# haoyuzhao123/CGRayTracing

Measured on NVIDIA B200. Metric: photons_per_s, higher is better.
Workload: dtype f64 decisions / f32 accumulators

## Files before the change

### cgraytracing_b200/csrc/cgrt_build.cuh

```cuda
#pragma once
#include "cgrt_device.cuh"

namespace cgrt {

#define RS_THREADS 256
#define RS_ITEMS 16
#define RS_TILE (RS_THREADS * RS_ITEMS)

template <typename K>
__global__ void __launch_bounds__(RS_THREADS) rs_hist_kernel(const K *__restrict__ keys, int64_t n, int shift, uint32_t *__restrict__ counts, int ntiles) {
    __shared__ uint32_t h[256];
    h[threadIdx.x] = 0;
    __syncthreads();
    int64_t base = (int64_t)blockIdx.x * RS_TILE;
#pragma unroll 4
    for (int r = 0; r < RS_ITEMS; r++) {
        int64_t i = base + r * RS_THREADS + threadIdx.x;
        if (i < n) atomicAdd(&h[(uint32_t)(keys[i] >> shift) & 255u], 1u);
    }
    __syncthreads();
    counts[(size_t)threadIdx.x * ntiles + blockIdx.x] = h[threadIdx.x];
}

__global__ void __launch_bounds__(1024) rs_scan_kernel(uint32_t *__restrict__ counts, int64_t m) {
    __shared__ uint32_t warp_sums[32];
    __shared__ uint32_t carry;
    if (threadIdx.x == 0) carry = 0;
    __syncthreads();
    int lane = threadIdx.x & 31, wid = threadIdx.x >> 5;
    for (int64_t base = 0; base < m; base += 1024) {
        int64_t i = base + threadIdx.x;
        uint32_t v = (i < m) ? counts[i] : 0u;
        uint32_t x = v;
#pragma unroll
        for (int o = 1; o < 32; o <<= 1) {
            uint32_t y = __shfl_up_sync(0xffffffffu, x, o);
            if (lane >= o) x += y;
        }
        if (lane == 31) warp_sums[wid] = x;
        __syncthreads();
        if (wid == 0) {
            uint32_t s = warp_sums[lane];
#pragma unroll
            for (int o = 1; o < 32; o <<= 1) {
                uint32_t y = __shfl_up_sync(0xffffffffu, s, o);
                if (lane >= o) s += y;
            }
            warp_sums[lane] = s;
        }
        __syncthreads();
        uint32_t prefix = carry + (wid > 0 ? warp_sums[wid - 1] : 0u) + x - v;
        if (i < m) counts[i] = prefix;
        __syncthreads();
        if (threadIdx.x == 1023) carry = prefix + v;
        __syncthreads();
    }
}

template <typename K>
__global__ void __launch_bounds__(RS_THREADS) rs_scatter_kernel(const K *__restrict__ keys_in, const uint32_t *__restrict__ vals_in,
                                                                K *__restrict__ keys_out, uint32_t *__restrict__ vals_out, int64_t n, int shift,
                                                                const uint32_t *__restrict__ offsets, int ntiles, int first_pass) {
    __shared__ uint32_t running[256];
    __shared__ uint32_t warp_cnt[RS_THREADS / 32][256];
    const int lane = threadIdx.x & 31, wid = threadIdx.x >> 5;
    running[threadIdx.x] = offsets[(size_t)threadIdx.x * ntiles + blockIdx.x];
#pragma unroll
    for (int w = 0; w < RS_THREADS / 32; w++) warp_cnt[w][threadIdx.x] = 0;
    __syncthreads();
    int64_t base = (int64_t)blockIdx.x * RS_TILE;
    for (int r = 0; r < RS_ITEMS; r++) {
        int64_t i = base + r * RS_THREADS + threadIdx.x;
        bool valid = i < n;
        K k = valid ? keys_in[i] : (K)0;
        uint32_t v = valid ? (first_pass ? (uint32_t)i : vals_in[i]) : 0u;
        uint32_t dg = valid ? ((uint32_t)(k >> shift) & 255u) : 256u;
        uint32_t mask = __match_any_sync(0xffffffffu, dg);
        uint32_t rank = __popc(mask & ((1u << lane) - 1u));
        if (valid && rank == 0) warp_cnt[wid][dg] = __popc(mask);
        __syncthreads();
        if (valid) {
            uint32_t pos = running[dg] + rank;
            for (int w = 0; w < wid; w++) pos += warp_cnt[w][dg];
            keys_out[pos] = k;
            vals_out[pos] = v;
        }
        __syncthreads();
        {
            uint32_t s = 0;
#pragma unroll
            for (int w = 0; w < RS_THREADS / 32; w++) { s += warp_cnt[w][threadIdx.x]; warp_cnt[w][threadIdx.x] = 0; }
            running[threadIdx.x] += s;
        }
        __syncthreads();
    }
}

__device__ __forceinline__ uint32_t float_flip(float f) {
    uint32_t u = __float_as_uint(f);
    return (u & 0x80000000u) ? ~u : (u | 0x80000000u);
}
__device__ __forceinline__ float float_unflip(uint32_t u) {
    return __uint_as_float((u & 0x80000000u) ? (u & 0x7fffffffu) : ~u);
}

__global__ void lbvh_bounds_kernel(const double *__restrict__ tri9, int n, uint32_t *__restrict__ bounds) {
    int i = blockIdx.x * blockDim.x + threadIdx.x;
    float c[3] = {3.0e38f, 3.0e38f, 3.0e38f}, C[3] = {-3.0e38f, -3.0e38f, -3.0e38f};
    if (i < n) {
        const double *t = tri9 + (size_t)i * 9;
        for (int a = 0; a < 3; a++) {
            float m = (float)((t[a] + t[3 + a] + t[6 + a]) * (1.0 / 3.0));
            c[a] = m; C[a] = m;
        }
    }
    for (int a = 0; a < 3; a++) {
        float lo = c[a], hi = C[a];
        for (int o = 16; o > 0; o >>= 1) {
            lo = fminf(lo, __shfl_xor_sync(0xffffffffu, lo, o));
            hi = fmaxf(hi, __shfl_xor_sync(0xffffffffu, hi, o));
        }
        if ((threadIdx.x & 31) == 0) {
            atomicMin(&bounds[a], float_flip(lo));
            atomicMax(&bounds[3 + a], float_flip(hi));
        }
    }
}

__device__ __forceinline__ uint32_t expand10(uint32_t v) {
    v = (v * 0x00010001u) & 0xFF0000FFu;
    v = (v * 0x00000101u) & 0x0F00F00Fu;
    v = (v * 0x00000011u) & 0xC30C30C3u;
    v = (v * 0x00000005u) & 0x49249249u;
    return v;
}

__global__ void lbvh_morton_kernel(const double *__restrict__ tri9, int n, const uint32_t *__restrict__ bounds, uint64_t *__restrict__ keys) {
    int i = blockIdx.x * blockDim.x + threadIdx.x;
    if (i >= n) return;
    const double *t = tri9 + (size_t)i * 9;
    uint32_t q[3];
    for (int a = 0; a < 3; a++) {
        float lo = float_unflip(bounds[a]), hi = float_unflip(bounds[3 + a]);
        float m = (float)((t[a] + t[3 + a] + t[6 + a]) * (1.0 / 3.0));
        float ext = hi - lo;
        float u = ext > 0.f ? (m - lo) / ext : 0.f;
        u = fminf(fmaxf(u * 1024.f, 0.f), 1023.f);
        q[a] = (uint32_t)u;
    }
    keys[i] = (uint64_t)((expand10(q[0]) << 2) | (expand10(q[1]) << 1) | expand10(q[2]));
}

__global__ void lbvh_leaves_kernel(const double *__restrict__ tri9, const uint32_t *__restrict__ perm, int n, TriRec *__restrict__ tris,
                                   int *__restrict__ tri_id, float *__restrict__ box ) {
    int k = blockIdx.x * blockDim.x + threadIdx.x;
    if (k >= n) return;
    uint32_t src = perm[k];
    const double *t = tri9 + (size_t)src * 9;
    d3 pa = mk(t[0], t[1], t[2]), pb = mk(t[3], t[4], t[5]), pc = mk(t[6], t[7], t[8]);
    d3 e1 = pa - pb, e2 = pa - pc;
    d3 nn = normalize(cross(pa - pb, pa - pc));
    TriRec R;
    R.pa[0] = pa.x; R.pa[1] = pa.y; R.pa[2] = pa.z;
    R.e1[0] = e1.x; R.e1[1] = e1.y; R.e1[2] = e1.z;
    R.e2[0] = e2.x; R.e2[1] = e2.y; R.e2[2] = e2.z;
    R.n[0] = nn.x; R.n[1] = nn.y; R.n[2] = nn.z;
    tris[k] = R;
    tri_id[k] = (int)src;
    float *b = box + (size_t)(n - 1 + k) * 6;
    const double pad = CGRT_BOX_PAD;
    for (int a = 0; a < 3; a++) {
        double lo = fmin(fmin(t[a], t[3 + a]), t[6 + a]), hi = fmax(fmax(t[a], t[3 + a]), t[6 + a]);
        b[a] = __double2float_rd(lo - pad - 1e-7 * fabs(lo));
        b[3 + a] = __double2float_ru(hi + pad + 1e-7 * fabs(hi));
    }
}

__device__ __forceinline__ int lbvh_delta(const uint64_t *__restrict__ keys, int n, int i, int j) {
    if (j < 0 || j >= n) return -1;
    uint64_t a = keys[i], b = keys[j];
    if (a == b) return 64 + __clz((uint32_t)i ^ (uint32_t)j);
    return __clzll((long long)(a ^ b));
}

__global__ void lbvh_hierarchy_kernel(const uint64_t *__restrict__ keys, int n, int *__restrict__ left, int *__restrict__ right, int *__restrict__ parent) {
    int i = blockIdx.x * blockDim.x + threadIdx.x;
    if (i >= n - 1) return;
    int d = (lbvh_delta(keys, n, i, i + 1) - lbvh_delta(keys, n, i, i - 1)) >= 0 ? 1 : -1;
    int dmin = lbvh_delta(keys, n, i, i - d);
    int lmax = 2;
    while (lbvh_delta(keys, n, i, i + lmax * d) > dmin) lmax <<= 1;
    int l = 0;
    for (int t = lmax >> 1; t >= 1; t >>= 1)
        if (lbvh_delta(keys, n, i, i + (l + t) * d) > dmin) l += t;
    int j = i + l * d;
    int dnode = lbvh_delta(keys, n, i, j);
    int s = 0;
    int t = l;
    do {
        t = (t + 1) >> 1;
        if (lbvh_delta(keys, n, i, i + (s + t) * d) > dnode) s += t;
    } while (t > 1);
    int gamma = i + s * d + min(d, 0);
    int lo = min(i, j), hi = max(i, j);
    int lc = (lo == gamma) ? (n - 1 + gamma) : gamma;
    int rc = (hi == gamma + 1) ? (n - 1 + gamma + 1) : (gamma + 1);
    left[i] = lc;
    right[i] = rc;
    parent[lc] = i;
    parent[rc] = i;
    if (i == 0) parent[0] = -1;
}

__global__ void lbvh_refit_kernel(int n, const int *__restrict__ left, const int *__restrict__ right, const int *__restrict__ parent,
                                  float *__restrict__ box, unsigned int *__restrict__ flags) {
    int k = blockIdx.x * blockDim.x + threadIdx.x;
    if (k >= n) return;
    int node = parent[n - 1 + k];
    while (node >= 0) {
        unsigned int old = atomicAdd(&flags[node], 1u);
        if (old == 0) return;
        __threadfence();
        const volatile float *a = box + (size_t)left[node] * 6;
        const volatile float *b = box + (size_t)right[node] * 6;
        float *o = box + (size_t)node * 6;
        for (int c = 0; c < 3; c++) {
            o[c] = fminf(a[c], b[c]);
            o[3 + c] = fmaxf(a[3 + c], b[3 + c]);
        }
        __threadfence();
        node = parent[node];
    }
}

__device__ __forceinline__ float lbvh_box_area(const float *__restrict__ b) {
    const float dx = b[3] - b[0], dy = b[4] - b[1], dz = b[5] - b[2];
    return dx * dy + dy * dz + dz * dx;
}
__global__ void lbvh_collapse_kernel(int n, int begin, int end, const int *__restrict__ left, const int *__restrict__ right, const float *__restrict__ box,
                                     int *__restrict__ queue, int *__restrict__ counter, BvhNode4 *__restrict__ nodes4) {
    int w = begin + blockIdx.x * blockDim.x + threadIdx.x;
    if (w >= end) return;
    const int b = queue[w];
    int c[4];
    int nc = 2;
    c[0] = left[b]; c[1] = right[b]; c[2] = -1; c[3] = -1;
    while (nc < 4) {
        int pick = -1;
        float best = -1.f;
        for (int j = 0; j < nc; j++) {
            if (c[j] >= n - 1) continue;
            float a = lbvh_box_area(box + (size_t)c[j] * 6);
            if (a > best) { best = a; pick = j; }
        }
        if (pick < 0) break;
        const int e = c[pick];
        c[pick] = left[e];
        c[nc++] = right[e];
    }
    for (int i = 1; i < nc; i++) {
        int v = c[i], j = i - 1;
        while (j >= 0 && c[j] > v) { c[j + 1] = c[j]; j--; }
        c[j + 1] = v;
    }
    BvhNode4 N;
    for (int j = 0; j < 4; j++) {
        if (j < nc) {
            const float *bb = box + (size_t)c[j] * 6;
            N.lox[j] = bb[0]; N.loy[j] = bb[1]; N.loz[j] = bb[2];
            N.hix[j] = bb[3]; N.hiy[j] = bb[4]; N.hiz[j] = bb[5];
            if (c[j] >= n - 1) {
                N.child[j] = ~(c[j] - (n - 1));
            } else {
                const int at = atomicAdd(counter, 1);
                queue[at] = c[j];
                N.child[j] = at;
            }
        } else {
            N.lox[j] = N.loy[j] = N.loz[j] = 3.0e38f;
            N.hix[j] = N.hiy[j] = N.hiz[j] = -3.0e38f;
            N.child[j] = CGRT_NO_CHILD;
        }
        N.pad[j] = 0;
    }
    nodes4[w] = N;
}

__global__ void bump_triangles_kernel(const double *__restrict__ height, int H, int W, double tex_px, double tex_pz, double lenx, double leny,
                                      double plane_y, double *__restrict__ tri9) {
    const int step = 3;
    int nj = W / step - 1, ni = H / step - 1;
    int idx = blockIdx.x * blockDim.x + threadIdx.x;
    if (idx >= ni * nj) return;
    int i = idx / nj, j = idx % nj;
    double x1 = tex_px + lenx * j * step / W;
    double x2 = tex_px + lenx * (j + 1) * step / W;
    double y1 = tex_pz + leny * i * step / H;
    double y2 = tex_pz + leny * (i + 1) * step / H;
    double ha = height[(size_t)(i * step) * W + j * step] + plane_y;
    double hb = height[(size_t)(i * step) * W + (j + 1) * step] + plane_y;
    double hc = height[(size_t)((i + 1) * step) * W + j * step] + plane_y;
    double hd = height[(size_t)((i + 1) * step) * W + (j + 1) * step] + plane_y;
    double *o = tri9 + (size_t)idx * 18;
    o[0] = x1; o[1] = ha; o[2] = y1;  o[3] = x2; o[4] = hb; o[5] = y1;  o[6] = x1; o[7] = hc; o[8] = y2;
    o[9] = x2; o[10] = hd; o[11] = y2;  o[12] = x2; o[13] = hb; o[14] = y1;  o[15] = x1; o[16] = hc; o[17] = y2;
}

__global__ void texture_stage_kernel(const uint8_t *__restrict__ rgb, int64_t ntexel, uchar4 *__restrict__ out) {
    int64_t i = (int64_t)blockIdx.x * blockDim.x + threadIdx.x;
    if (i >= ntexel) return;
    out[i] = make_uchar4(rgb[3 * i], rgb[3 * i + 1], rgb[3 * i + 2], 255);
}

}
```

### cgraytracing_b200/csrc/cgrt_device.cuh

```cuda
#pragma once
#include <cuda_runtime.h>
#include <stdint.h>

namespace cgrt {

struct d3 {
    double x, y, z;
};
__host__ __device__ __forceinline__ d3 mk(double x, double y, double z) { d3 r; r.x = x; r.y = y; r.z = z; return r; }
__host__ __device__ __forceinline__ d3 operator+(d3 a, d3 b) { return mk(a.x + b.x, a.y + b.y, a.z + b.z); }
__host__ __device__ __forceinline__ d3 operator-(d3 a, d3 b) { return mk(a.x - b.x, a.y - b.y, a.z - b.z); }
__host__ __device__ __forceinline__ d3 operator-(d3 a) { return mk(-a.x, -a.y, -a.z); }
__host__ __device__ __forceinline__ d3 operator*(d3 a, double f) { return mk(a.x * f, a.y * f, a.z * f); }
__host__ __device__ __forceinline__ d3 operator*(d3 a, d3 b) { return mk(a.x * b.x, a.y * b.y, a.z * b.z); }
__host__ __device__ __forceinline__ double dot(d3 a, d3 b) { return a.x * b.x + a.y * b.y + a.z * b.z; }
__host__ __device__ __forceinline__ d3 cross(d3 a, d3 b) {
    return mk(a.y * b.z - a.z * b.y, a.z * b.x - a.x * b.z, a.x * b.y - a.y * b.x);
}
__host__ __device__ __forceinline__ d3 normalize(d3 a) {
    double len = sqrt(a.x * a.x + a.y * a.y + a.z * a.z);
    if (len > 0) {
        a.x *= 1 / len;
        a.y *= 1 / len;
        a.z *= 1 / len;
    }
    return a;
}
__host__ __device__ __forceinline__ double det3(d3 a, d3 b, d3 c) {
    return (a.x * b.y * c.z + b.x * c.y * a.z + c.x * a.y * b.z - a.x * c.y * b.z - b.x * a.y * c.z - c.x * b.y * a.z);
}
__host__ __device__ __forceinline__ double max3(double a, double b, double c) {
    if (a > b && a > c) return a;
    else if (b > c) return b;
    else return c;
}

#define CGRT_EPS 1e-4
#define CGRT_INF 1e10
#define CGRT_PI 3.14159265358979

enum { PASS_EYE = 0, PASS_PHOTON = 1, PASS_BEZIER = 2, PASS_SPPM_EYE = 3 };

struct Philox {
    uint32_t k0, k1, c0, c1, c2, c3;
    uint32_t buf[4];
    int idx;
    __host__ __device__ __forceinline__ void init(uint64_t seed, uint32_t pass, uint64_t path, uint32_t dim) {
        k0 = (uint32_t)seed;
        k1 = (uint32_t)(seed >> 32) + pass;
        c0 = (uint32_t)path;
        c1 = (uint32_t)(path >> 32);
        c2 = dim;
        c3 = 0;
        idx = 4;
    }
    __host__ __device__ __forceinline__ void block() {
        uint32_t a0 = c0, a1 = c1, a2 = c2, a3 = c3, x0 = k0, x1 = k1;
#pragma unroll
        for (int r = 0; r < 10; r++) {
#ifdef __CUDA_ARCH__
            uint32_t h0 = __umulhi(0xD2511F53u, a0), l0 = 0xD2511F53u * a0;
            uint32_t h1 = __umulhi(0xCD9E8D57u, a2), l1 = 0xCD9E8D57u * a2;
#else
            uint64_t p0 = (uint64_t)0xD2511F53u * a0, p1 = (uint64_t)0xCD9E8D57u * a2;
            uint32_t h0 = (uint32_t)(p0 >> 32), l0 = (uint32_t)p0, h1 = (uint32_t)(p1 >> 32), l1 = (uint32_t)p1;
#endif
            uint32_t n0 = h1 ^ a1 ^ x0, n2 = h0 ^ a3 ^ x1;
            a0 = n0; a1 = l1; a2 = n2; a3 = l0;
            x0 += 0x9E3779B9u;
            x1 += 0xBB67AE85u;
        }
        buf[0] = a0; buf[1] = a1; buf[2] = a2; buf[3] = a3;
        c3++;
        idx = 0;
    }
    __host__ __device__ __forceinline__ double u01() {
        if (idx == 4) block();
        uint32_t w = buf[0];
        w = idx == 1 ? buf[1] : w;
        w = idx == 2 ? buf[2] : w;
        w = idx == 3 ? buf[3] : w;
        idx++;
        return (double)(w >> 1) * (1.0 / 2147483648.0);
    }
};

#define CGRT_MAX_REJECT 64
__host__ __device__ __forceinline__ void sincos2pi(double v, double &s_out, double &c_out) {
    double t = 4.0 * v;
    int k = (int)(t + 0.5);
    double r = t - (double)k;
    double x = r * 1.5707963267948966;
    double z = x * x;
    double ps = -1.66666666666666324348e-01 + z * (8.33333333332248946124e-03 + z * (-1.98412698298579493134e-04 + z * (2.75573137070700676789e-06 +
                z * (-2.50507602534068634195e-08 + z * 1.58969099521155010221e-10))));
    double sn = x + x * z * ps;
    double pc = 4.16666666666666019037e-02 + z * (-1.38888888888741095749e-03 + z * (2.48015872894767294178e-05 + z * (-2.75573143513906633035e-07 +
                z * (2.08757232129817482790e-09 + z * -1.13596475577881948265e-11))));
    double cs = 1.0 - 0.5 * z + z * z * pc;
    int q = k & 3;
    s_out = q == 0 ? sn : (q == 1 ? cs : (q == 2 ? -sn : -cs));
    c_out = q == 0 ? cs : (q == 1 ? -sn : (q == 2 ? -cs : sn));
}
__host__ __device__ __forceinline__ d3 sample_sphere(Philox &g) {
    double z = 1.0 - 2.0 * g.u01();
    double sn, cs;
    sincos2pi(g.u01(), sn, cs);
    double r = sqrt(1.0 - z * z);
    return mk(r * cs, r * sn, z);
}
__host__ __device__ __forceinline__ d3 sample_halfsphere(Philox &g, d3 dir) {
    d3 s = sample_sphere(g);
    if (dot(s, dir) < 0) s = -s;
    return s;
}
__host__ __device__ __forceinline__ d3 sample_circle(Philox &g, double radius) {
    double x = 0, y = 0;
    for (int it = 0; it < CGRT_MAX_REJECT; it++) {
        x = g.u01() * 2.0 - 1;
        y = g.u01() * 2.0 - 1;
        if (x * x + y * y < 1) break;
    }
    return mk(x, y, 0) * radius;
}

enum { OBJ_SPHERE = 0, OBJ_PLANE = 1, OBJ_MESH = 2, OBJ_BEZIER = 3 };
enum { MAT_DIFFUSE = 0, MAT_MIRROR = 1, MAT_GLASS = 2 };

#define CGRT_MAX_OBJECTS 12
#define CGRT_MAX_BVH 4
#define CGRT_MAX_TEX 4
#define CGRT_MAX_BEZIER 2
#define CGRT_MAX_CP 7

#define CGRT_NO_CHILD ((int)0x80000000)
struct __align__(16) BvhNode4 {
    float lox[4], loy[4], loz[4], hix[4], hiy[4], hiz[4];
    int child[4];
    int pad[4];
};
struct __align__(16) TriRec {
    double pa[3], e1[3], e2[3], n[3];
};

struct ObjDev {
    int kind, material, tex, bvh, objtype, aux;
    double a[3];
    double b[3];
    double r, r2;
    double col[3];
    double refl, transp;
};
struct BvhDev {
    const BvhNode4 *nodes4;
    const TriRec *tris;
    const int *tri_id;
    int ntris;
    int root_is_leaf;
    double orient_sign;
    float root_lo[3], root_hi[3];
    int f32_ok;
    int pad;
};
struct TexDev {
    const uchar4 *texels;
    int W, H, isbump, pad;
    double n[3], p[3], lenx, leny;
};
struct BezDev {
    int ncp, pad;
    double cp[CGRT_MAX_CP][3];
    double pos[3];
    double box[6];
    double umin_r2;
    double C[CGRT_MAX_CP], Cm[CGRT_MAX_CP];
};
struct SceneDev {
    int nobj, nbvh, ntex, nbez;
    int nplane, nsphere, ndeferred;
    unsigned char plane_ix[CGRT_MAX_OBJECTS], sphere_ix[CGRT_MAX_OBJECTS], deferred_ix[CGRT_MAX_OBJECTS];
    ObjDev obj[CGRT_MAX_OBJECTS];
    BvhDev bvh[CGRT_MAX_BVH];
    TexDev tex[CGRT_MAX_TEX];
    BezDev bez[CGRT_MAX_BEZIER];
};

struct Hit {
    double t;
    d3 n;
    int obj;
    int prim;
};

struct TravCounters {
    unsigned long long node_visits, tri_tests;
};

__device__ __forceinline__ bool tri_intersect(const TriRec *T, d3 o, d3 d, double &t) {
    const double2 *tq = reinterpret_cast<const double2 *>(T);
    double2 a0 = __ldg(tq), a1 = __ldg(tq + 1), a2 = __ldg(tq + 2), a3 = __ldg(tq + 3);
    double a4 = __ldg(reinterpret_cast<const double *>(tq + 4));
    d3 pa = mk(a0.x, a0.y, a1.x);
    d3 e1 = mk(a1.y, a2.x, a2.y);
    d3 e2 = mk(a3.x, a3.y, a4);
    d3 s = pa - o;
    double det1 = det3(d, e1, e2);
    if (det1 == 0.0 || det1 != det1) return false;
    double det3v = det3(d, s, e2);
    double det4v = det3(d, e1, s);
    bool pos = det1 > 0.0;
    if (!(det3v == 0.0 || ((det3v > 0.0) == pos))) return false;
    if (!(det4v == 0.0 || ((det4v > 0.0) == pos))) return false;
    double sum = det3v + det4v;
    if (pos ? !(sum <= det1) : !(sum >= det1)) return false;
    double det2 = det3(s, e1, e2);
    double q = det2 / det1;
    if (!(q > 0.0)) return false;
    t = q;
    return true;
}

#define CGRT_F32_BOUND 64.0
#define CGRT_BOX_PAD 8e-5

struct SlabRay {
    float ox, oy, oz, ix, iy, iz;
    d3 o, id;
    bool exact;
};
__device__ __forceinline__ SlabRay make_slab_ray(d3 o, d3 d, bool f32_ok) {
    SlabRay r;
    r.exact = !(f32_ok && fabs(o.x) <= CGRT_F32_BOUND && fabs(o.y) <= CGRT_F32_BOUND && fabs(o.z) <= CGRT_F32_BOUND);
    r.o = o;
    r.id = mk(0, 0, 0);
    if (r.exact) r.id = mk(1.0 / d.x, 1.0 / d.y, 1.0 / d.z);
    r.ox = (float)o.x; r.oy = (float)o.y; r.oz = (float)o.z;
    r.ix = 1.0f / (float)d.x; r.iy = 1.0f / (float)d.y; r.iz = 1.0f / (float)d.z;
    return r;
}
__device__ __forceinline__ bool slab64(float lx, float ly, float lz, float hx, float hy, float hz, const SlabRay &r, double tmax, float &tnear) {
    double tx0 = ((double)lx - r.o.x) * r.id.x, tx1 = ((double)hx - r.o.x) * r.id.x;
    double ty0 = ((double)ly - r.o.y) * r.id.y, ty1 = ((double)hy - r.o.y) * r.id.y;
    double tz0 = ((double)lz - r.o.z) * r.id.z, tz1 = ((double)hz - r.o.z) * r.id.z;
    double tn = fmax(fmax(fmin(tx0, tx1), fmin(ty0, ty1)), fmax(fmin(tz0, tz1), 0.0));
    double tf = fmin(fmin(fmax(tx0, tx1), fmax(ty0, ty1)), fmin(fmax(tz0, tz1), tmax));
    tnear = (float)tn;
    return tn <= tf;
}
__device__ __forceinline__ bool slab32(float lx, float ly, float lz, float hx, float hy, float hz, const SlabRay &r, float tmax_up, float &tnear) {
    float tx0 = (lx - r.ox) * r.ix, tx1 = (hx - r.ox) * r.ix;
    float ty0 = (ly - r.oy) * r.iy, ty1 = (hy - r.oy) * r.iy;
    float tz0 = (lz - r.oz) * r.iz, tz1 = (hz - r.oz) * r.iz;
    float tn = fmaxf(fmaxf(fminf(tx0, tx1), fminf(ty0, ty1)), fmaxf(fminf(tz0, tz1), 0.0f));
    float tf = fminf(fminf(fmaxf(tx0, tx1), fmaxf(ty0, ty1)), fminf(fmaxf(tz0, tz1), tmax_up));
    tnear = tn;
    return tn <= tf;
}
__device__ __forceinline__ bool slab_any(float lx, float ly, float lz, float hx, float hy, float hz, const SlabRay &r, double tmax, float tmax_up,
                                         float &tnear) {
    return r.exact ? slab64(lx, ly, lz, hx, hy, hz, r, tmax, tnear) : slab32(lx, ly, lz, hx, hy, hz, r, tmax_up, tnear);
}
__device__ __forceinline__ bool root_box_hit(const BvhDev &B, d3 o, d3 d, double tmax) {
    if (!B.f32_ok) {
        SlabRay r = make_slab_ray(o, d, false);
        float tn;
        return slab_any(B.root_lo[0], B.root_lo[1], B.root_lo[2], B.root_hi[0], B.root_hi[1], B.root_hi[2], r, tmax, __double2float_ru(tmax), tn);
    }
    const float ox = (float)o.x, oy = (float)o.y, oz = (float)o.z;
    const float ix = 1.0f / (float)d.x, iy = 1.0f / (float)d.y, iz = 1.0f / (float)d.z;
    const float pad = 1e-6f * (fmaxf(fmaxf(fabsf(ox), fabsf(oy)), fabsf(oz)) + (float)CGRT_F32_BOUND);
    const float tx0 = (B.root_lo[0] - pad - ox) * ix, tx1 = (B.root_hi[0] + pad - ox) * ix;
    const float ty0 = (B.root_lo[1] - pad - oy) * iy, ty1 = (B.root_hi[1] + pad - oy) * iy;
    const float tz0 = (B.root_lo[2] - pad - oz) * iz, tz1 = (B.root_hi[2] + pad - oz) * iz;
    const float tn = fmaxf(fmaxf(fminf(tx0, tx1), fminf(ty0, ty1)), fmaxf(fminf(tz0, tz1), 0.0f));
    const float tf = fminf(fminf(fmaxf(tx0, tx1), fmaxf(ty0, ty1)), fminf(fmaxf(tz0, tz1), __double2float_ru(tmax)));
    return tn <= tf;
}

#ifndef CGRT_BVH_STACK
#define CGRT_BVH_STACK 160
#endif
__device__ __forceinline__ float f4c(const float4 &v, int j) { return j == 0 ? v.x : (j == 1 ? v.y : (j == 2 ? v.z : v.w)); }
__device__ __forceinline__ void cswap(unsigned int &a, unsigned int &b) {
    const unsigned int lo = min(a, b), hi = max(a, b);
    a = lo; b = hi;
}

template <bool COUNT, bool F32ONLY>
__device__ __forceinline__ bool bvh4_closest(const BvhDev &B, d3 o, d3 d, double tmax, double &t_out, int &leaf_out, TravCounters *tc) {
    double t0 = 0.0;
    SlabRay R;
    float ox, oy, oz, ix, iy, iz;
    if (F32ONLY) {
        d3 ob = o;
        if (!(fabs(o.x) <= CGRT_F32_BOUND && fabs(o.y) <= CGRT_F32_BOUND && fabs(o.z) <= CGRT_F32_BOUND)) {
            const double jx = 1.0 / d.x, jy = 1.0 / d.y, jz = 1.0 / d.z;
            const double tx0 = ((double)B.root_lo[0] - o.x) * jx, tx1 = ((double)B.root_hi[0] - o.x) * jx;
            const double ty0 = ((double)B.root_lo[1] - o.y) * jy, ty1 = ((double)B.root_hi[1] - o.y) * jy;
            const double tz0 = ((double)B.root_lo[2] - o.z) * jz, tz1 = ((double)B.root_hi[2] - o.z) * jz;
            const double tn = fmax(fmax(fmin(tx0, tx1), fmin(ty0, ty1)), fmax(fmin(tz0, tz1), 0.0));
            const double tf = fmin(fmin(fmax(tx0, tx1), fmax(ty0, ty1)), fmin(fmax(tz0, tz1), tmax));
            if (!(tn <= tf)) { t_out = tmax; leaf_out = -1; return false; }
            t0 = tn * (1.0 - 1e-12);
            ob = o + d * t0;
        }
        ox = (float)ob.x; oy = (float)ob.y; oz = (float)ob.z;
        ix = 1.0f / (float)d.x; iy = 1.0f / (float)d.y; iz = 1.0f / (float)d.z;
        R.exact = false;
    } else {
        R = make_slab_ray(o, d, B.f32_ok != 0);
        ox = R.ox; oy = R.oy; oz = R.oz; ix = R.ix; iy = R.iy; iz = R.iz;
    }
    const float cx = -(ox * ix), cy = -(oy * iy), cz = -(oz * iz);
    const int sxo = ix < 0.f ? 3 : 0, syo = iy < 0.f ? 3 : 0, szo = iz < 0.f ? 3 : 0;
    double best = tmax;
    float best_up = __double2float_ru(tmax - t0);
    int best_leaf = -1;
    int stack[CGRT_BVH_STACK];
    int sp = 0;
    int node = B.root_is_leaf ? ~0 : 0;
    for (;;) {
        if (node >= 0) {
            const float4 *q = reinterpret_cast<const float4 *>(B.nodes4 + node);
            const int4 ch = __ldg(reinterpret_cast<const int4 *>(q + 6));
            if (COUNT) tc->node_visits += 4;
            unsigned int key[4];
            if (!F32ONLY && R.exact) {
                const float4 lx = __ldg(q), ly = __ldg(q + 1), lz = __ldg(q + 2), hx = __ldg(q + 3), hy = __ldg(q + 4), hz = __ldg(q + 5);
#pragma unroll
                for (int j = 0; j < 4; j++) {
                    float tn;
                    const bool h = slab64(f4c(lx, j), f4c(ly, j), f4c(lz, j), f4c(hx, j), f4c(hy, j), f4c(hz, j), R, best, tn);
                    key[j] = h ? ((__float_as_uint(tn) & ~3u) | (unsigned int)j) : 0xffffffffu;
                }
            } else {
                const float4 nx = __ldg(q + sxo), fx = __ldg(q + 3 - sxo), ny = __ldg(q + 1 + syo), fy = __ldg(q + 4 - syo);
                const float4 nz = __ldg(q + 2 + szo), fz = __ldg(q + 5 - szo);
#pragma unroll
                for (int j = 0; j < 4; j++) {
                    const float tn = fmaxf(fmaxf(fmaf(f4c(nx, j), ix, cx), fmaf(f4c(ny, j), iy, cy)), fmaxf(fmaf(f4c(nz, j), iz, cz), 0.0f));
                    const float tf = fminf(fminf(fmaf(f4c(fx, j), ix, cx), fmaf(f4c(fy, j), iy, cy)), fminf(fmaf(f4c(fz, j), iz, cz), best_up));
                    key[j] = (tn <= tf) ? ((__float_as_uint(tn) & ~3u) | (unsigned int)j) : 0xffffffffu;
                }
            }
            if (ch.z == CGRT_NO_CHILD) key[2] = 0xffffffffu;
            if (ch.w == CGRT_NO_CHILD) key[3] = 0xffffffffu;
            cswap(key[0], key[1]); cswap(key[2], key[3]); cswap(key[0], key[2]); cswap(key[1], key[3]); cswap(key[1], key[2]);
            if (key[0] == 0xffffffffu) {
                if (sp == 0) break;
                node = stack[--sp];
            } else {
                int c[4];
#pragma unroll
                for (int k = 0; k < 4; k++) {
                    const unsigned int s1 = (key[k] & 1u) << 5, s2 = (key[k] & 2u) << 4;
                    const unsigned int lo = __funnelshift_rc((unsigned int)ch.x, (unsigned int)ch.y, s1);
                    const unsigned int hi = __funnelshift_rc((unsigned int)ch.z, (unsigned int)ch.w, s1);
                    c[k] = (int)__funnelshift_rc(lo, hi, s2);
                }
                if (key[3] != 0xffffffffu) stack[sp++] = c[3];
                if (key[2] != 0xffffffffu) stack[sp++] = c[2];
                if (key[1] != 0xffffffffu) stack[sp++] = c[1];
                node = c[0];
            }
        } else {
            const int leaf = ~node;
            if (COUNT) tc->tri_tests++;
            double t;
            if (tri_intersect(B.tris + leaf, o, d, t) && t < best) {
                best = t;
                best_up = __double2float_ru(t - t0);
                best_leaf = leaf;
            }
            if (sp == 0) break;
            node = stack[--sp];
        }
    }
    t_out = best;
    leaf_out = best_leaf;
    return best_leaf >= 0;
}

__device__ __forceinline__ bool box_any_face_hit(const double *b, d3 o, d3 d) {
    const double e = 1e-4;
    double xmax = b[0], xmin = b[1], ymax = b[2], ymin = b[3], zmax = b[4], zmin = b[5];
    double t; d3 p;
    t = (xmax - o.x) / d.x; p = o + d * t;
    if (t > 0 && p.y >= ymin - e && p.y <= ymax + e && p.z >= zmin - e && p.z <= zmax + e) return true;
    t = (xmin - o.x) / d.x; p = o + d * t;
    if (t > 0 && p.y >= ymin - e && p.y <= ymax + e && p.z >= zmin - e && p.z <= zmax + e) return true;
    t = (ymax - o.y) / d.y; p = o + d * t;
    if (t > 0 && p.x >= xmin - e && p.x <= xmax + e && p.z >= zmin - e && p.z <= zmax + e) return true;
    t = (ymin - o.y) / d.y; p = o + d * t;
    if (t > 0 && p.x >= xmin - e && p.x <= xmax + e && p.z >= zmin - e && p.z <= zmax + e) return true;
    t = (zmax - o.z) / d.z; p = o + d * t;
    if (t > 0 && p.x >= xmin - e && p.x <= xmax + e && p.y >= ymin - e && p.y <= ymax + e) return true;
    t = (zmin - o.z) / d.z; p = o + d * t;
    if (t > 0 && p.x >= xmin - e && p.x <= xmax + e && p.y >= ymin - e && p.y <= ymax + e) return true;
    return false;
}

__host__ __device__ inline void bez_binomials(int ncp, double *C, double *Cm) {
    int n = ncp - 1;
    for (int i = 0; i < CGRT_MAX_CP; i++) { C[i] = 0.0; Cm[i] = 0.0; }
    C[0] = 1.0; Cm[0] = 1.0;
    for (int i = 1; i <= n; i++) C[i] = C[i - 1] * (double)(n - i + 1) / (double)i;
    for (int i = 1; i <= n - 1; i++) Cm[i] = Cm[i - 1] * (double)(n - i) / (double)i;
}
__device__ __forceinline__ void bez_eval(const BezDev &Z, double u, d3 &P, d3 &dP) {
    int n = Z.ncp - 1;
    const double *C = Z.C, *Cm = Z.Cm;
    double pu[CGRT_MAX_CP], pv[CGRT_MAX_CP];
    pu[0] = 1.0; pv[0] = 1.0;
    for (int i = 1; i <= n; i++) { pu[i] = pu[i - 1] * u; pv[i] = pv[i - 1] * (1.0 - u); }
    P = mk(0, 0, 0); dP = mk(0, 0, 0);
    for (int i = 0; i <= n; i++) {
        double b = C[i] * pv[n - i] * pu[i];
        double db = 0.0;
        if (i > 0) db += Cm[i - 1] * pv[n - i] * pu[i - 1] * (double)i;
        if (i < n) db -= Cm[i] * pv[n - 1 - i] * pu[i] * (double)(n - i);
        d3 c = mk(Z.cp[i][0], Z.cp[i][1], Z.cp[i][2]);
        P = P + c * b;
        dP = dP + c * db;
    }
}

__device__ __forceinline__ d3 bez_F(const BezDev &Z, d3 par, d3 o, d3 d, d3 &P, d3 &dP, double &s, double &c) {
    bez_eval(Z, par.y, P, dP);
    sincos(par.z, &s, &c);
    d3 surf = mk(P.z * s, P.y, P.z * c);
    return o + d * par.x - mk(Z.pos[0], Z.pos[1], Z.pos[2]) - surf;
}

#define CGRT_BEZ_SEEDS 16
#ifndef CGRT_BEZ_MAXIT
#define CGRT_BEZ_MAXIT 40
#endif
__device__ __forceinline__ bool bezier_newton_seed(const BezDev &Z, d3 o, d3 d, int seed, double &t_out, d3 &nrm_out) {
    const d3 pos = mk(Z.pos[0], Z.pos[1], Z.pos[2]);
    const double rmax = Z.box[0] - Z.pos[0];
    const double tc = dot(pos - o, d);
    const double tlo = fmax(tc - 2.0 * rmax - (Z.box[2] - Z.box[3]), 0.0), thi = tc + 2.0 * rmax + (Z.box[2] - Z.box[3]);
    const int iu = seed >> 2, it = seed & 3;
    double u0 = (iu + 0.5) * 0.25;
    double t0 = tlo + (thi - tlo) * (it + 0.5) * 0.25;
    d3 pt = o + d * t0 - pos;
    double theta = (pt.z < 0) ? 3.14159265 + atan(pt.x / pt.z) : atan(pt.x / pt.z);
    d3 par = mk(t0, u0, theta);
    d3 P, dP;
    double s, c;
    d3 F = bez_F(Z, par, o, d, P, dP, s, c);
    int iter = 0;
    while (sqrt(dot(F, F)) > 1e-6 && iter < CGRT_BEZ_MAXIT) {
        iter++;
        d3 a = d;
        d3 b = mk(-s * dP.z, -dP.y, -c * dP.z);
        d3 cc = mk(-c * P.z, 0.0, s * P.z);
        double D = det3(a, b, cc);
        if (D < 1e-4 && D > -1e-4) {
            par = mk(par.x + 0.037, par.y + 0.029 * ((iter & 1) ? 1 : -1), par.z + 0.041);
            F = bez_F(Z, par, o, d, P, dP, s, c);
            continue;
        }
        const double iD = 1.0 / D;
        d3 ra = mk((b.y * cc.z - b.z * cc.y) * iD, (cc.y * a.z - cc.z * a.y) * iD, (a.y * b.z - a.z * b.y) * iD);
        d3 rb = mk((cc.x * b.z - cc.z * b.x) * iD, (a.x * cc.z - a.z * cc.x) * iD, (b.x * a.z - b.z * a.x) * iD);
        d3 rc = mk((b.x * cc.y - cc.x * b.y) * iD, (cc.x * a.y - cc.y * a.x) * iD, (a.x * b.y - a.y * b.x) * iD);
        d3 step = ra * F.x + rb * F.y + rc * F.z;
        par = par - step;
        F = bez_F(Z, par, o, d, P, dP, s, c);
    }
    if (!(sqrt(dot(F, F)) < 1e-4 && par.x > 0 && par.y <= 1 && par.y >= 0)) return false;
    t_out = par.x;
    d3 g = normalize(dP);
    nrm_out = mk(g.y * s, -g.z, g.y * c);
    return true;
}
__device__ __forceinline__ void bezier_finish(const BezDev &Z, d3 o, d3 d, double &len, d3 &nrm) {
    const d3 pos = mk(Z.pos[0], Z.pos[1], Z.pos[2]);
    nrm = nrm * ((dot(nrm, d) < 0) ? 1.0 : -1.0);
    double newt = Z.box[2] - o.y;
    if (newt > 0.1) {
        newt = newt / d.y;
        d3 np = o + d * newt;
        if ((np.x - pos.x) * (np.x - pos.x) + (np.z - pos.z) * (np.z - pos.z) <= Z.umin_r2) {
            len = newt;
            nrm = mk(0, 1, 0);
        }
    }
}
__device__ bool bezier_intersect(const BezDev &Z, d3 o, d3 d, double &len, d3 &nrm) {
    if (!box_any_face_hit(Z.box, o, d)) return false;
    bool flag = false;
    len = CGRT_INF;
    for (int seed = 0; seed < CGRT_BEZ_SEEDS; seed++) {
        double t; d3 nv;
        if (bezier_newton_seed(Z, o, d, seed, t, nv) && t < len) { len = t; nrm = nv; flag = true; }
    }
    bezier_finish(Z, o, d, len, nrm);
    return flag;
}
__device__ __forceinline__ bool bezier_intersect_halfwarp(const BezDev &Z, d3 o, d3 d, double &len, d3 &nrm) {
    const unsigned int lane = threadIdx.x & 31u, half_mask = (lane < 16u) ? 0x0000ffffu : 0xffff0000u;
    if (!box_any_face_hit(Z.box, o, d)) return false;
    double t = CGRT_INF; d3 nv = mk(0, 0, 0);
    bool ok = bezier_newton_seed(Z, o, d, (int)(lane & 15u), t, nv);
    if (!ok) t = CGRT_INF;
    int who = ok ? (int)(lane & 15u) : 16;
#pragma unroll
    for (int off = 8; off >= 1; off >>= 1) {
        double t2 = __shfl_xor_sync(half_mask, t, off);
        int w2 = __shfl_xor_sync(half_mask, who, off);
        if (t2 < t || (t2 == t && w2 < who)) { t = t2; who = w2; }
    }
    if (who >= 16) return false;
    const int src = (int)(lane & 16u) + who;
    nv.x = __shfl_sync(half_mask, nv.x, src); nv.y = __shfl_sync(half_mask, nv.y, src); nv.z = __shfl_sync(half_mask, nv.z, src);
    len = t; nrm = nv;
    bezier_finish(Z, o, d, len, nrm);
    return true;
}

template <int BLOCK>
struct TraceShared {
    double ox[BLOCK], oy[BLOCK], oz[BLOCK], dx[BLOCK], dy[BLOCK], dz[BLOCK];
    double lim[BLOCK];
    int leaf[BLOCK];
    double near_in[BLOCK];
    int id_in[BLOCK];
    unsigned short list[BLOCK];
    unsigned int count;
    unsigned int scratch[8];
};

__device__ __forceinline__ double next_up(double x) { return __longlong_as_double(__double_as_longlong(x) + 1); }

__device__ __forceinline__ double plane_len(const ObjDev &O, d3 o, d3 d) {
    d3 n = mk(O.b[0], O.b[1], O.b[2]);
    d3 dd = mk(O.a[0], O.a[1], O.a[2]) - o;
    double num = dot(dd, n);
    if (num == 0.0) return 0.0;
    return num / dot(d, n);
}

struct HitAcc {
    double nearest;
    int id, prim;
    d3 nrm;
};

__device__ __forceinline__ void plane_take(const SceneDev &S, int i, double len, HitAcc &A) {
    if (len > 0 && len < A.nearest) {
        const ObjDev &O = S.obj[i];
        A.id = i; A.nearest = len; A.nrm = mk(O.b[0], O.b[1], O.b[2]); A.prim = -1;
    }
}
__device__ __forceinline__ void analytic_phase(const SceneDev &S, d3 o, d3 d, HitAcc &A) {
    A.nearest = CGRT_INF; A.id = -1; A.prim = -1; A.nrm = mk(0, 0, 0);
    int k = 0;
    for (; k + 3 <= S.nplane; k += 3) {
        const int i0 = S.plane_ix[k], i1 = S.plane_ix[k + 1], i2 = S.plane_ix[k + 2];
        const double l0 = plane_len(S.obj[i0], o, d), l1 = plane_len(S.obj[i1], o, d), l2 = plane_len(S.obj[i2], o, d);
        plane_take(S, i0, l0, A); plane_take(S, i1, l1, A); plane_take(S, i2, l2, A);
    }
    for (; k < S.nplane; k++) {
        const int i = S.plane_ix[k];
        plane_take(S, i, plane_len(S.obj[i], o, d), A);
    }
    for (k = 0; k < S.nsphere; k++) {
        const int i = S.sphere_ix[k];
        const ObjDev &O = S.obj[i];
        d3 l = mk(O.a[0], O.a[1], O.a[2]) - o;
        double tca = dot(l, d);
        double l2 = dot(l, l);
        if (!(tca < 0 && l2 > O.r2)) {
            double d2 = dot(l, l) - tca * tca;
            if (!(d2 > O.r2)) {
                double thc = sqrt(O.r2 - d2);
                double t0 = tca - thc, t1 = tca + thc;
                double len = (t0 < 0) ? t1 : t0;
                if (len < A.nearest || (len == A.nearest && i < A.id)) {
                    d3 p = o + d * len;
                    A.id = i; A.nearest = len; A.prim = -1;
                    A.nrm = normalize(p - mk(O.a[0], O.a[1], O.a[2]));
                }
            }
        }
    }
}
__device__ __forceinline__ bool is_deferred(const ObjDev &O) { return O.bvh >= 0 || O.kind == OBJ_BEZIER; }
__device__ __forceinline__ bool deferred_wanted(const SceneDev &S, int i, d3 o, d3 d, const HitAcc &A, double &lim) {
    const ObjDev &O = S.obj[i];
    lim = (A.id > i) ? next_up(A.nearest) : A.nearest;
    if (O.kind == OBJ_BEZIER) return box_any_face_hit(S.bez[O.aux].box, o, d);
    if (O.kind == OBJ_PLANE) {
        double len = plane_len(O, o, d);
        if (!(len > 0)) return false;
        lim = len < lim ? len : lim;
    }
    return root_box_hit(S.bvh[O.bvh], o, d, lim);
}
__device__ __forceinline__ void bvh_merge(const SceneDev &S, int i, int leaf, double t, HitAcc &A) {
    const ObjDev &O = S.obj[i];
    const BvhDev &B = S.bvh[O.bvh];
    const TriRec &T = B.tris[leaf];
    d3 nv = mk(T.n[0], T.n[1], T.n[2]) * B.orient_sign;
    if (O.kind == OBJ_MESH && O.objtype == 2) nv = nv * ((nv.y > 0) ? 1.0 : -1.0);
    A.id = i; A.nearest = t; A.nrm = nv; A.prim = B.tri_id[leaf];
}

template <bool COUNT, bool BEZ, bool F32 = false>
__device__ __forceinline__ bool deferred_resolve(const SceneDev &S, int i, d3 o, d3 d, double lim, HitAcc &A, TravCounters *tc) {
    const ObjDev &O = S.obj[i];
    if (O.kind == OBJ_BEZIER) {
        if (BEZ) {
            double len; d3 nv;
            if (bezier_intersect(S.bez[O.aux], o, d, len, nv) && (len < A.nearest || (len == A.nearest && i < A.id))) {
                A.id = i; A.nearest = len; A.nrm = nv; A.prim = -1;
                return true;
            }
        }
        return false;
    }
    double t; int leaf;
    if (!bvh4_closest<COUNT, F32>(S.bvh[O.bvh], o, d, lim, t, leaf, tc)) return false;
    bvh_merge(S, i, leaf, t, A);
    return true;
}

template <int BLOCK, bool COUNT, bool F32 = false>
__device__ __forceinline__ bool closest_hit_block(const SceneDev &S, bool active, d3 o, d3 d, Hit &h, TraceShared<BLOCK> &sm, TravCounters *tc) {
    HitAcc A;
    A.nearest = CGRT_INF; A.id = -1; A.prim = -1; A.nrm = mk(0, 0, 0);
    if (active) analytic_phase(S, o, d, A);
    const int tid = threadIdx.x, lane = tid & 31;
    for (int i = 0; i < S.nobj; i++) {
        const ObjDev &O = S.obj[i];
        if (!is_deferred(O)) continue;
        double lim = 0;
        bool want = active && deferred_wanted(S, i, o, d, A, lim);
        if (tid == 0) sm.count = 0;
        __syncthreads();
        unsigned int mask = __ballot_sync(0xffffffffu, want);
        unsigned int base = 0;
        if (mask) {
            if (lane == __ffs(mask) - 1) base = atomicAdd(&sm.count, (unsigned int)__popc(mask));
            base = __shfl_sync(0xffffffffu, base, __ffs(mask) - 1);
        }
        if (want) {
            sm.list[base + __popc(mask & ((1u << lane) - 1u))] = (unsigned short)tid;
            sm.ox[tid] = o.x; sm.oy[tid] = o.y; sm.oz[tid] = o.z;
            sm.dx[tid] = d.x; sm.dy[tid] = d.y; sm.dz[tid] = d.z;
            sm.lim[tid] = lim;
            sm.near_in[tid] = A.nearest; sm.id_in[tid] = A.id;
        }
        __syncthreads();
        if (O.kind == OBJ_BEZIER) {
            const int half = tid >> 4, nhalf = BLOCK / 16, cnt = (int)sm.count;
            for (int r = 0; r * nhalf < cnt; r++) {
                const int e = r * nhalf + half;
                const bool live = e < cnt;
                const int s = live ? sm.list[e] : 0;
                double len; d3 nv;
                bool hit = live && bezier_intersect_halfwarp(S.bez[O.aux], mk(sm.ox[s], sm.oy[s], sm.oz[s]), mk(sm.dx[s], sm.dy[s], sm.dz[s]), len, nv);
                if (live) __syncwarp((tid & 16) ? 0xffff0000u : 0x0000ffffu);
                hit = hit && (len < sm.near_in[s] || (len == sm.near_in[s] && i < sm.id_in[s]));
                if (live && (tid & 15) == 0) {
                    sm.leaf[s] = hit ? 1 : 0;
                    if (hit) { sm.lim[s] = len; sm.ox[s] = nv.x; sm.oy[s] = nv.y; sm.oz[s] = nv.z; sm.id_in[s] = -1; }
                }
            }
        } else if (tid < (int)sm.count) {
            int s = sm.list[tid];
            HitAcc R;
            R.nearest = sm.near_in[s]; R.id = sm.id_in[s]; R.prim = -1; R.nrm = mk(0, 0, 0);
            bool hit = deferred_resolve<COUNT, false, F32>(S, i, mk(sm.ox[s], sm.oy[s], sm.oz[s]), mk(sm.dx[s], sm.dy[s], sm.dz[s]), sm.lim[s], R, tc);
            sm.leaf[s] = hit ? 1 : 0;
            if (hit) {
                sm.lim[s] = R.nearest; sm.ox[s] = R.nrm.x; sm.oy[s] = R.nrm.y; sm.oz[s] = R.nrm.z; sm.id_in[s] = R.prim;
            }
        }
        __syncthreads();
        if (want && sm.leaf[tid]) { A.id = i; A.nearest = sm.lim[tid]; A.nrm = mk(sm.ox[tid], sm.oy[tid], sm.oz[tid]); A.prim = sm.id_in[tid]; }
        __syncthreads();
    }
    h.obj = A.id; h.t = A.nearest; h.n = A.nrm; h.prim = A.prim;
    return A.id >= 0;
}

__device__ __forceinline__ d3 surface_color(const SceneDev &S, int obj, d3 point) {
    const ObjDev &O = S.obj[obj];
    d3 flat = mk(O.col[0], O.col[1], O.col[2]);
    if (O.kind != OBJ_PLANE || O.tex < 0) return flat;
    const TexDev &T = S.tex[O.tex];
    const double texteps = 1e-2;
    d3 n = mk(T.n[0], T.n[1], T.n[2]);
    d3 dd = point - mk(T.p[0], T.p[1], T.p[2]);
    dd = dd - n * dot(dd, n);
    int r, c;
    if (dd.x < texteps && dd.x > -texteps) {
        if (0 < dd.y && dd.y < T.lenx && 0 < dd.z && dd.z < T.leny) {
            r = (int)floor(dd.y / T.lenx * T.H);
            c = (int)floor(dd.z / T.leny * T.W);
        } else return flat;
    } else if (dd.y < texteps && dd.y > -texteps) {
        if (0 < dd.x && dd.x < T.lenx && 0 < dd.z && dd.z < T.leny) {
            c = (int)floor(dd.x / T.lenx * T.W);
            r = (int)floor(dd.z / T.leny * T.H);
        } else return flat;
    } else if (dd.z < texteps && dd.z > -texteps) {
        if (0 < dd.x && dd.x < T.lenx && 0 < dd.y && dd.y < T.leny) {
            c = (int)floor(dd.x / T.lenx * T.W);
            r = T.H - 1 - (int)floor(dd.y / T.leny * T.H);
        } else return flat;
    } else {
        return flat;
    }
    r = r < 0 ? 0 : (r >= T.H ? T.H - 1 : r);
    c = c < 0 ? 0 : (c >= T.W ? T.W - 1 : c);
    uchar4 tx = __ldg(T.texels + (size_t)r * T.W + c);
    return mk((double)tx.x / 256.0, (double)tx.y / 256.0, (double)tx.z / 256.0);
}

__host__ __device__ __forceinline__ int cell_floor_div(double num, double den, double inv_den) {
    double q = num * inv_den;
    double f = floor(q);
    double tol = fabs(q) * 1e-15 + 1e-300;
    if (q - f < tol || (f + 1.0) - q < tol) f = floor(num / den);
    return (int)f;
}
__host__ __device__ __forceinline__ void cell_coord(d3 p, double celllength, double inv, int &ix, int &iy, int &iz) {
    ix = cell_floor_div(p.x - (-35.0), celllength, inv);
    iy = cell_floor_div(p.y - (-35.0), celllength, inv);
    iz = cell_floor_div(p.z - (-15.0), celllength, inv);
}
__host__ __device__ __forceinline__ uint32_t cell_hash(int ix, int iy, int iz, uint32_t hashsize) {
    return (((uint32_t)ix * 73856093u) ^ ((uint32_t)iy * 19349663u) ^ ((uint32_t)iz * 83492791u)) % hashsize;
}

}
```

Measured before the change: 1.003 billion.

## Quantize BVH4 child bounds to 8-bit per axis in 64-byte nodes

Replaces the 128-byte wide BVH node holding full float child boxes with a 64-byte compressed node: a per-axis float origin and power-of-two scale plus 8-bit conservative lo/hi offsets per child. Traversal decodes the bytes with FMAs, folding scale into the slab computation and using directed rounding on the exact path, so each node costs four 16-byte loads instead of seven. This halves node memory traffic and cache footprint but adds byte-extraction ALU work and looser boxes that may cause extra node visits. Inverse directions are clamped so the scaled slab terms stay finite.

```diff
diff --git a/cgraytracing_b200/csrc/cgrt_build.cuh b/cgraytracing_b200/csrc/cgrt_build.cuh
--- a/cgraytracing_b200/csrc/cgrt_build.cuh
+++ b/cgraytracing_b200/csrc/cgrt_build.cuh
@@ -264,11 +264,11 @@
         c[j + 1] = v;
     }
     BvhNode4 N;
+    float lo[4][3], hi[4][3];
     for (int j = 0; j < 4; j++) {
         if (j < nc) {
             const float *bb = box + (size_t)c[j] * 6;
-            N.lox[j] = bb[0]; N.loy[j] = bb[1]; N.loz[j] = bb[2];
-            N.hix[j] = bb[3]; N.hiy[j] = bb[4]; N.hiz[j] = bb[5];
+            for (int a = 0; a < 3; a++) { lo[j][a] = bb[a]; hi[j][a] = bb[3 + a]; }
             if (c[j] >= n - 1) {
                 N.child[j] = ~(c[j] - (n - 1));
             } else {
@@ -277,12 +277,10 @@
                 N.child[j] = at;
             }
         } else {
-            N.lox[j] = N.loy[j] = N.loz[j] = 3.0e38f;
-            N.hix[j] = N.hiy[j] = N.hiz[j] = -3.0e38f;
             N.child[j] = CGRT_NO_CHILD;
         }
-        N.pad[j] = 0;
-    }
+    }
+    bvhq_encode(N, nc, lo, hi);
     nodes4[w] = N;
 }
 
diff --git a/cgraytracing_b200/csrc/cgrt_bvhq.h b/cgraytracing_b200/csrc/cgrt_bvhq.h
--- /dev/null
+++ b/cgraytracing_b200/csrc/cgrt_bvhq.h
@@ -0,0 +1,66 @@
+#pragma once
+#include <math.h>
+#include <stdint.h>
+
+#if defined(__CUDACC__)
+#define CGRT_HD __host__ __device__ __forceinline__
+#else
+#define CGRT_HD inline
+#endif
+
+namespace cgrt {
+
+#define CGRT_NO_CHILD ((int)0x80000000)
+struct alignas(16) BvhNode4 {
+    float org[3];
+    float scale[3];
+    uint32_t qlo[3], qhi[3];
+    int child[4];
+};
+static_assert(sizeof(BvhNode4) == 64, "BvhNode4 is 64 bytes");
+
+#define CGRT_BVHQ_EMIN (-100)
+#define CGRT_BVHQ_INV_MAX 0x1p100f
+
+CGRT_HD float bvhq_byte(uint32_t w, int j) { return (float)((w >> (8 * j)) & 255u); }
+
+CGRT_HD void bvhq_axis(float org, float scale, float inv, float c, float &s, float &k) {
+    s = scale * inv;
+    k = fmaf(org, inv, c);
+}
+CGRT_HD float bvhq_t(uint32_t w, int j, float s, float k) { return fmaf(bvhq_byte(w, j), s, k); }
+
+CGRT_HD void bvhq_encode(BvhNode4 &N, int nc, const float lo[][3], const float hi[][3]) {
+    const double widen = 1.0 / 4503599627370496.0;
+    for (int a = 0; a < 3; a++) {
+        float ulo = lo[0][a], uhi = hi[0][a];
+        for (int j = 1; j < nc; j++) {
+            ulo = fminf(ulo, lo[j][a]);
+            uhi = fmaxf(uhi, hi[j][a]);
+        }
+        double ext = (double)uhi - (double)ulo;
+        ext = ext + ext * widen;
+        int e;
+        frexp(ext / 255.0, &e);
+        if (e < CGRT_BVHQ_EMIN) e = CGRT_BVHQ_EMIN;
+        while (ceil(ldexp(ext, -e)) > 255.0) e++;
+        while (e > CGRT_BVHQ_EMIN && ceil(ldexp(ext, 1 - e)) <= 255.0) e--;
+        N.org[a] = ulo;
+        N.scale[a] = (float)ldexp(1.0, e);
+        uint32_t wl = 0, wh = 0;
+        for (int j = 0; j < 4; j++) {
+            uint32_t ql = 255u, qh = 0u;
+            if (j < nc) {
+                const double dl = (double)lo[j][a] - (double)ulo, dh = (double)hi[j][a] - (double)ulo;
+                ql = (uint32_t)floor(ldexp(dl - dl * widen, -e));
+                qh = (uint32_t)ceil(ldexp(dh + dh * widen, -e));
+            }
+            wl |= ql << (8 * j);
+            wh |= qh << (8 * j);
+        }
+        N.qlo[a] = wl;
+        N.qhi[a] = wh;
+    }
+}
+
+}
diff --git a/cgraytracing_b200/csrc/cgrt_device.cuh b/cgraytracing_b200/csrc/cgrt_device.cuh
--- a/cgraytracing_b200/csrc/cgrt_device.cuh
+++ b/cgraytracing_b200/csrc/cgrt_device.cuh
@@ -1,6 +1,8 @@
 #pragma once
 #include <cuda_runtime.h>
 #include <stdint.h>
+
+#include "cgrt_bvhq.h"
 
 namespace cgrt {
 
@@ -133,12 +135,6 @@
 #define CGRT_MAX_BEZIER 2
 #define CGRT_MAX_CP 7
 
-#define CGRT_NO_CHILD ((int)0x80000000)
-struct __align__(16) BvhNode4 {
-    float lox[4], loy[4], loz[4], hix[4], hiy[4], hiz[4];
-    int child[4];
-    int pad[4];
-};
 struct __align__(16) TriRec {
     double pa[3], e1[3], e2[3], n[3];
 };
@@ -280,7 +276,6 @@
 #ifndef CGRT_BVH_STACK
 #define CGRT_BVH_STACK 160
 #endif
-__device__ __forceinline__ float f4c(const float4 &v, int j) { return j == 0 ? v.x : (j == 1 ? v.y : (j == 2 ? v.z : v.w)); }
 __device__ __forceinline__ void cswap(unsigned int &a, unsigned int &b) {
     const unsigned int lo = min(a, b), hi = max(a, b);
     a = lo; b = hi;
@@ -311,8 +306,11 @@
         R = make_slab_ray(o, d, B.f32_ok != 0);
         ox = R.ox; oy = R.oy; oz = R.oz; ix = R.ix; iy = R.iy; iz = R.iz;
     }
+    ix = fminf(fmaxf(ix, -CGRT_BVHQ_INV_MAX), CGRT_BVHQ_INV_MAX);
+    iy = fminf(fmaxf(iy, -CGRT_BVHQ_INV_MAX), CGRT_BVHQ_INV_MAX);
+    iz = fminf(fmaxf(iz, -CGRT_BVHQ_INV_MAX), CGRT_BVHQ_INV_MAX);
     const float cx = -(ox * ix), cy = -(oy * iy), cz = -(oz * iz);
-    const int sxo = ix < 0.f ? 3 : 0, syo = iy < 0.f ? 3 : 0, szo = iz < 0.f ? 3 : 0;
+    const bool nx = ix < 0.f, ny = iy < 0.f, nz = iz < 0.f;
     double best = tmax;
     float best_up = __double2float_ru(tmax - t0);
     int best_leaf = -1;
@@ -321,25 +319,34 @@
     int node = B.root_is_leaf ? ~0 : 0;
     for (;;) {
         if (node >= 0) {
-            const float4 *q = reinterpret_cast<const float4 *>(B.nodes4 + node);
-            const int4 ch = __ldg(reinterpret_cast<const int4 *>(q + 6));
+            const uint4 *q = reinterpret_cast<const uint4 *>(B.nodes4 + node);
+            const uint4 w0 = __ldg(q), w1 = __ldg(q + 1), w2 = __ldg(q + 2);
+            const int4 ch = __ldg(reinterpret_cast<const int4 *>(q + 3));
+            const float orgx = __uint_as_float(w0.x), orgy = __uint_as_float(w0.y), orgz = __uint_as_float(w0.z);
+            const float scx = __uint_as_float(w0.w), scy = __uint_as_float(w1.x), scz = __uint_as_float(w1.y);
             if (COUNT) tc->node_visits += 4;
             unsigned int key[4];
             if (!F32ONLY && R.exact) {
-                const float4 lx = __ldg(q), ly = __ldg(q + 1), lz = __ldg(q + 2), hx = __ldg(q + 3), hy = __ldg(q + 4), hz = __ldg(q + 5);
 #pragma unroll
                 for (int j = 0; j < 4; j++) {
                     float tn;
-                    const bool h = slab64(f4c(lx, j), f4c(ly, j), f4c(lz, j), f4c(hx, j), f4c(hy, j), f4c(hz, j), R, best, tn);
+                    const bool h = slab64(__fmaf_rd(bvhq_byte(w1.z, j), scx, orgx), __fmaf_rd(bvhq_byte(w1.w, j), scy, orgy),
+                                          __fmaf_rd(bvhq_byte(w2.x, j), scz, orgz), __fmaf_ru(bvhq_byte(w2.y, j), scx, orgx),
+                                          __fmaf_ru(bvhq_byte(w2.z, j), scy, orgy), __fmaf_ru(bvhq_byte(w2.w, j), scz, orgz), R, best, tn);
                     key[j] = h ? ((__float_as_uint(tn) & ~3u) | (unsigned int)j) : 0xffffffffu;
                 }
             } else {
-                const float4 nx = __ldg(q + sxo), fx = __ldg(q + 3 - sxo), ny = __ldg(q + 1 + syo), fy = __ldg(q + 4 - syo);
-                const float4 nz = __ldg(q + 2 + szo), fz = __ldg(q + 5 - szo);
+                float sx, sy, sz, kx, ky, kz;
+                bvhq_axis(orgx, scx, ix, cx, sx, kx);
+                bvhq_axis(orgy, scy, iy, cy, sy, ky);
+                bvhq_axis(orgz, scz, iz, cz, sz, kz);
+                const uint32_t qnx = nx ? w2.y : w1.z, qfx = nx ? w1.z : w2.y;
+                const uint32_t qny = ny ? w2.z : w1.w, qfy = ny ? w1.w : w2.z;
+                const uint32_t qnz = nz ? w2.w : w2.x, qfz = nz ? w2.x : w2.w;
 #pragma unroll
                 for (int j = 0; j < 4; j++) {
-                    const float tn = fmaxf(fmaxf(fmaf(f4c(nx, j), ix, cx), fmaf(f4c(ny, j), iy, cy)), fmaxf(fmaf(f4c(nz, j), iz, cz), 0.0f));
-                    const float tf = fminf(fminf(fmaf(f4c(fx, j), ix, cx), fmaf(f4c(fy, j), iy, cy)), fminf(fmaf(f4c(fz, j), iz, cz), best_up));
+                    const float tn = fmaxf(fmaxf(bvhq_t(qnx, j, sx, kx), bvhq_t(qny, j, sy, ky)), fmaxf(bvhq_t(qnz, j, sz, kz), 0.0f));
+                    const float tf = fminf(fminf(bvhq_t(qfx, j, sx, kx), bvhq_t(qfy, j, sy, ky)), fminf(bvhq_t(qfz, j, sz, kz), best_up));
                     key[j] = (tn <= tf) ? ((__float_as_uint(tn) & ~3u) | (unsigned int)j) : 0xffffffffu;
                 }
             }
```

Result: no change. 1.006 billion, median of 6 (+0.3%).
